# GuidoManni/BodySLAM

Measured on AMD Instinct MI355X. Metric: frames/sec depth+pose+back-proj, 640x480 seq, higher is better.
Workload: dtype f16

## Files before the change

### bodyslam_amd/_lib.py

```python
from __future__ import annotations

import ctypes as C
import os
from typing import Optional

import torch

_HERE = os.path.dirname(os.path.abspath(__file__))
LIB_PATH = os.environ.get("BODYSLAM_HIP_LIB") or os.path.join(_HERE, "libbodyslam_hip.so")

F32, F16, BF16 = 0, 1, 2
F64 = 3
ACT_NONE, ACT_RELU, ACT_GELU, ACT_SOFTPLUS, ACT_SOFTPLUS_FAST = 0, 1, 2, 3, 4
OUT_PLAIN, OUT_SHUFFLE, OUT_QKV = 0, 1, 2

_TORCH2BS = {torch.float32: F32, torch.float16: F16, torch.bfloat16: BF16}
BS2TORCH = {F32: torch.float32, F16: torch.float16, BF16: torch.bfloat16}


class BodySlamHipError(RuntimeError):
    pass


class GemmDesc(C.Structure):
# ... 70 lines not shown
    "bs_odo_p2p_prepare": [C.c_void_p, C.c_int32, C.c_int32, C.c_int32, C.c_double, C.c_void_p, C.c_void_p],
    "bs_odo_p2p_target": [C.c_void_p, C.c_int32, C.c_int32, C.c_int32, C.c_void_p, C.c_void_p, C.c_void_p],
    "bs_odo_p2p_accumulate": [C.c_void_p, C.c_void_p, C.c_int32, C.c_int32, C.c_void_p, C.c_void_p, C.c_double, C.c_double, C.c_void_p, C.c_void_p,
                              C.c_void_p],
    "bs_odo_p2p_step": [C.c_void_p, C.c_void_p, C.c_int32, C.c_int32, C.c_int32, C.c_void_p, C.c_void_p, C.c_int32, C.c_double, C.c_double, C.c_void_p,
                        C.c_void_p, C.c_void_p],
    "bs_tsdf_extract": [C.c_void_p, C.c_int32, C.c_void_p, C.c_void_p, C.c_int32, C.c_void_p, C.c_int32, C.c_int32, C.c_double, C.c_void_p, C.c_void_p,
                        C.c_void_p, C.c_void_p, C.c_void_p, C.c_void_p],
    "bs_tsdf_mesh": [C.c_void_p, C.c_int32, C.c_void_p, C.c_void_p, C.c_int32, C.c_void_p, C.c_int32, C.c_int32, C.c_double, C.c_void_p, C.c_int32] + [C.c_void_p] * 7,
    "bs_tsdf_raycast": [C.c_void_p, C.c_void_p, C.c_int32, C.c_int32, C.c_int32, C.c_double, C.c_double, C.c_void_p, C.c_void_p, C.c_int32, C.c_void_p,
                        C.c_int32, C.c_int32, C.c_double, C.c_double, C.c_void_p, C.c_void_p, C.c_void_p, C.c_void_p, C.c_void_p],
    "bs_attractor_step": [C.c_void_p] * 4 + [C.c_int32] * 8 + [C.c_void_p],
    "bs_add_resized": [C.c_void_p] * 3 + [C.c_int32] * 7 + [C.c_void_p],
    "bs_mlp2": [C.c_void_p, C.c_int32] + [C.c_void_p] * 5 + [C.c_int32] * 6 + [C.c_void_p],
    "bs_mlp2_add": [C.c_void_p] * 7 + [C.c_int32] * 10 + [C.c_void_p],
    "bs_projector_level": [C.c_void_p] * 10 + [C.c_int32] * 9 + [C.c_void_p],
    "bs_logbinom_depth": [C.c_void_p] * 8 + [C.c_int32] * 5 + [C.c_float, C.c_float, C.c_int32, C.c_void_p],
    "bs_logbinom_depth_ex": [C.c_void_p] * 7 + [C.c_int32] + [C.c_void_p] * 2 + [C.c_int32] * 5 + [C.c_float, C.c_float, C.c_int32, C.c_void_p],
    "bs_small_attention": [C.c_void_p, C.c_void_p, C.c_int32, C.c_int32, C.c_int32, C.c_int32, C.c_void_p],
    "bs_route_argmax": [C.c_void_p, C.c_int32, C.c_void_p, C.c_int32, C.c_void_p],
    "bs_postprocess_depth": [C.c_void_p] * 3 + [C.c_int32] * 6 + [C.c_void_p],
    "bs_cyclepose_im2col": [C.c_void_p] * 3 + [C.c_int32] * 4 + [C.c_void_p],
    "bs_cyclepose_im2col_window": [C.c_void_p] * 3 + [C.c_int32] * 8 + [C.c_void_p],
    "bs_instnorm_relu_nhwc": [C.c_void_p] * 4 + [C.c_int32] * 3 + [C.c_float, C.c_int32, C.c_void_p],
    "bs_avgpool_nhwc": [C.c_void_p, C.c_void_p, C.c_int32, C.c_int32, C.c_int32, C.c_void_p],
    "bs_cyclepose_head": [C.c_void_p] * 12 + [C.c_int32] * 3 + [C.c_void_p],
    "bs_backproject": [C.c_void_p, C.c_int32, C.c_int32, C.c_int32, C.c_void_p, C.c_double, C.c_double] + [C.c_void_p] * 6,
    "bs_pose_chain": [C.c_void_p, C.c_int32, C.c_void_p, C.c_void_p, C.c_void_p],
    "bs_pose_chain_from": [C.c_void_p, C.c_int32, C.c_void_p, C.c_void_p, C.c_void_p],
    "bs_pixel_to_3d": [C.c_void_p, C.c_int64, C.c_void_p, C.c_void_p, C.c_void_p],
    "bs_depth_metrics_workspace": [C.c_int32, C.c_int32, C.c_int32],
    "bs_depth_metrics": [C.c_void_p, C.c_void_p] + [C.c_int32] * 3 + [C.c_double, C.c_double, C.c_int32, C.c_double, C.c_void_p, C.c_int64,
                                                                       C.c_void_p, C.c_void_p],
    "bs_similarity_fit": [C.c_void_p, C.c_void_p, C.c_int64, C.c_int32, C.c_void_p, C.c_int64, C.c_void_p, C.c_void_p],
    "bs_trajectory_metrics": [C.c_void_p, C.c_void_p, C.c_void_p, C.c_int32, C.c_int64, C.c_int32, C.c_int32, C.c_int32, C.c_void_p, C.c_void_p],
    "bs_orb_pyramid": [C.c_void_p, C.c_int32, C.c_int32, C.c_int32, C.c_int32, C.c_void_p, C.c_int32, C.c_int64, C.c_void_p, C.c_void_p, C.c_void_p],
    "bs_orb_fast": [C.c_void_p, C.c_int32, C.c_int32, C.c_int32, C.c_void_p, C.c_int32, C.c_int64, C.c_void_p, C.c_void_p, C.c_void_p],
    "bs_orb_select": [C.c_void_p, C.c_void_p, C.c_void_p, C.c_int32, C.c_int32, C.c_int32, C.c_void_p, C.c_int32, C.c_int64, C.c_void_p,
                      C.c_void_p, C.c_void_p, C.c_void_p, C.c_void_p],
    "bs_orb_describe": [C.c_void_p, C.c_void_p, C.c_int32, C.c_int32, C.c_int32, C.c_void_p, C.c_int32, C.c_int64, C.c_void_p, C.c_void_p,
                        C.c_void_p, C.c_void_p, C.c_void_p, C.c_void_p, C.c_void_p, C.c_void_p],
    "bs_orb_match": [C.c_void_p, C.c_void_p, C.c_int32, C.c_void_p, C.c_void_p, C.c_void_p],
    "bs_orb_displacement": [C.c_void_p, C.c_void_p, C.c_void_p, C.c_void_p, C.c_void_p, C.c_int32, C.c_int32, C.c_int32, C.c_void_p, C.c_int32,
                            C.c_void_p, C.c_void_p],
    "bs_orb_lift": [C.c_void_p, C.c_void_p, C.c_void_p, C.c_int32, C.c_int32, C.c_int32, C.c_void_p, C.c_void_p, C.c_void_p],
    "bs_orb_match_pairs": [C.c_void_p, C.c_void_p, C.c_int32, C.c_void_p, C.c_int32, C.c_void_p, C.c_void_p, C.c_void_p],
# ... 474 lines not shown

def logbinom_depth(last, Eh, bins, w0_last, w2, b2, route, depth, B, H, W, He, We, min_temp, max_temp):
    check(load_library().bs_logbinom_depth(p(last), p(Eh), p(bins), p(w0_last), p(w2), p(b2), p(route), p(depth), B, H, W, He, We,
                                           min_temp, max_temp, dt(last), stream_ptr()), "bs_logbinom_depth")


def small_attention(qkv, out, B, S, nheads):
    check(load_library().bs_small_attention(p(qkv), p(out), B, S, nheads, dt(out), stream_ptr()), "bs_small_attention")


def route_argmax(logits, ld, route, B):
    check(load_library().bs_route_argmax(p(logits), ld, p(route), B, stream_ptr()), "bs_route_argmax")


def postprocess_depth(depth_net, depth_m, depth_u16, B, H, W, nh, nw, flip):
    check(load_library().bs_postprocess_depth(p(depth_net), p(depth_m), p(depth_u16), B, H, W, nh, nw, int(flip), stream_ptr()),
          "bs_postprocess_depth")


def cyclepose_im2col(frames, pairs, out, P, H, W):
    check(load_library().bs_cyclepose_im2col(p(frames), p(pairs), p(out), P, H, W, dt(out), stream_ptr()), "bs_cyclepose_im2col")


def instnorm_relu_nhwc(x, out, out_f32, scratch, P, HW, Cch, eps=1e-5):
    check(load_library().bs_instnorm_relu_nhwc(p(x), p(out), p(out_f32), p(scratch), P, HW, Cch, eps, dt(out), stream_ptr()),
          "bs_instnorm_relu_nhwc")


def avgpool_nhwc(x, out, P, HW, Cch):
    check(load_library().bs_avgpool_nhwc(p(x), p(out), P, HW, Cch, stream_ptr()), "bs_avgpool_nhwc")


def cyclepose_head(pooled, x2, w_skip_pool, w_skip_x2, b_skip, w1, b1, w2, b2, pose7, T, scratch, P, HW, Cch):
    check(load_library().bs_cyclepose_head(p(pooled), p(x2), p(w_skip_pool), p(w_skip_x2), p(b_skip), p(w1), p(b1), p(w2), p(b2),
                                           p(pose7), p(T), p(scratch), P, HW, Cch, stream_ptr()), "bs_cyclepose_head")


def backproject(depth_u16, K4, depth_scale, depth_trunc, poses, xyz, idx, count, scratch, B, H, W):
    Karr = (C.c_double * 4)(*[float(v) for v in K4])
    check(load_library().bs_backproject(p(depth_u16), B, H, W, C.cast(Karr, C.c_void_p), float(depth_scale), float(depth_trunc),
                                        p(poses), p(xyz), p(idx), p(count), p(scratch), stream_ptr()), "bs_backproject")


def pose_chain(t_rel, N, g0, g_abs):
    g0arr = None
    if g0 is not None:
        g0arr = C.cast((C.c_double * 16)(*[float(v) for v in g0]), C.c_void_p)
    check(load_library().bs_pose_chain(p(t_rel), N, g0arr, p(g_abs), stream_ptr()), "bs_pose_chain")
# ... 261 lines not shown
```

### bodyslam_amd/csrc/cyclepose.hip

```cpp
#include "common.h"

namespace bs {

constexpr int CP_CROP = 128;
constexpr int CP_K = 320;

template <typename T, bool SPLIT>
__global__ __launch_bounds__(256) void cp_im2col_kernel(const uint8_t* frames, const int32_t* pairs, T* out, int P, int H, int W,
                                                         int top, int left, int CH, int CW) {
    const int64_t total = (int64_t)P * CH * CW * 54;
    const int64_t gid = (int64_t)blockIdx.x * blockDim.x + threadIdx.x;
    if (gid >= total) return;
    const int slot = (int)(gid % 54);
    const int64_t m = gid / 54;
    T* row = out + m * (SPLIT ? 2 * CP_K : CP_K);
    if (slot >= 49) {
        const int k0 = 294 + (slot - 49) * 6;
        for (int i = 0; i < 6 && k0 + i < CP_K; ++i) {
            row[k0 + i] = T16<T>::from_f32(0.0f);
            if (SPLIT) row[CP_K + k0 + i] = T16<T>::from_f32(0.0f);
        }
        return;
    }
    const int x = (int)(m % CW);
// ... 1 lines not shown
    const int p = (int)(m / ((int64_t)CW * CH));
    const int ky = slot / 7, kx = slot - ky * 7;
    int yy = y + ky - 3, xx = x + kx - 3;
    yy = yy < 0 ? -yy : (yy >= CH ? 2 * CH - 2 - yy : yy);
    xx = xx < 0 ? -xx : (xx >= CW ? 2 * CW - 2 - xx : xx);
    const int f0 = pairs[2 * p], f1 = pairs[2 * p + 1];
    const uint8_t* p0 = frames + (((int64_t)f0 * H + top + yy) * W + left + xx) * 3;
    const uint8_t* p1 = frames + (((int64_t)f1 * H + top + yy) * W + left + xx) * 3;
    T* o = row + slot * 6;
#pragma unroll
    for (int c = 0; c < 3; ++c) {
        const float v0 = (__fdiv_rn((float)p0[c], 255.0f) - 0.5f) / 0.5f, v1 = (__fdiv_rn((float)p1[c], 255.0f) - 0.5f) / 0.5f;
        o[c] = T16<T>::from_f32(v0);
        o[3 + c] = T16<T>::from_f32(v1);
        if (SPLIT) {
            o[CP_K + c] = T16<T>::from_f32(v0 - T16<T>::to_f32(o[c]));
            o[CP_K + 3 + c] = T16<T>::from_f32(v1 - T16<T>::to_f32(o[3 + c]));
        }
    }
}

constexpr int IN_CHUNK = 256;

__global__ __launch_bounds__(256) void instnorm_stats_kernel(const float* x, float* part, int HW, int C, int nchunk) {
    const int p = blockIdx.y, ch = blockIdx.x;
    const int tpr = C >> 2, rps = 256 / tpr;
    const int c4 = (threadIdx.x % tpr) * 4, rg = threadIdx.x / tpr;
    const int r0 = ch * IN_CHUNK, r1 = min(HW, r0 + IN_CHUNK);
    const float* xp = x + ((int64_t)p * HW) * C + c4;
    __shared__ float red[256 * 4];
    __shared__ float mean_s[256];
    f32x4 s = {0, 0, 0, 0};
    for (int r = r0 + rg; r < r1; r += rps) {
        const f32x4 v = *reinterpret_cast<const f32x4*>(xp + (int64_t)r * C);
        s += v;
    }
    *reinterpret_cast<f32x4*>(red + threadIdx.x * 4) = s;
    __syncthreads();
    if (threadIdx.x < C) {
        const int c = threadIdx.x;
        float a = 0.f;
        for (int g = 0; g < rps; ++g) a += red[(g * tpr + (c >> 2)) * 4 + (c & 3)];
        mean_s[c] = a / (float)(r1 - r0);
    }
    __syncthreads();
    const f32x4 mu = *reinterpret_cast<const f32x4*>(mean_s + c4);
    f32x4 q = {0, 0, 0, 0};
    for (int r = r0 + rg; r < r1; r += rps) {
        const f32x4 v = *reinterpret_cast<const f32x4*>(xp + (int64_t)r * C) - mu;
        q += v * v;
    }
    __syncthreads();
    *reinterpret_cast<f32x4*>(red + threadIdx.x * 4) = q;
    __syncthreads();
    if (threadIdx.x < C) {
        const int c = threadIdx.x;
        float a = 0.f;
        for (int g = 0; g < rps; ++g) a += red[(g * tpr + (c >> 2)) * 4 + (c & 3)];
        float* o = part + (((int64_t)p * nchunk + ch) * 2) * C;
        o[c] = mean_s[c];
        o[C + c] = a;
    }
}

template <typename T, bool SPLIT>
__global__ __launch_bounds__(256) void instnorm_apply_kernel(const float* x, const float* part, T* out, float* out_f32, int HW, int C,
                                                              int nchunk, float eps) {
    const int p = blockIdx.y, ch = blockIdx.x;
    const int tpr = C >> 2, rps = 256 / tpr;
    const int c4 = (threadIdx.x % tpr) * 4, rg = threadIdx.x / tpr;
    const int r0 = ch * IN_CHUNK, r1 = min(HW, r0 + IN_CHUNK);
    __shared__ float mean_s[256], rstd_s[256];
    if (threadIdx.x < C) {
        const int c = threadIdx.x;
        const float* pp = part + ((int64_t)p * nchunk * 2) * C + c;
        float msum = 0.f;
        for (int k = 0; k < nchunk; ++k) msum += pp[(int64_t)k * 2 * C] * (float)(min(HW, (k + 1) * IN_CHUNK) - k * IN_CHUNK);
        const float mean = msum / (float)HW;
        float m2 = 0.f;
        for (int k = 0; k < nchunk; ++k) {
            const float d = pp[(int64_t)k * 2 * C] - mean;
            m2 += pp[(int64_t)k * 2 * C + C] + d * d * (float)(min(HW, (k + 1) * IN_CHUNK) - k * IN_CHUNK);
        }
        mean_s[c] = mean;
        rstd_s[c] = 1.0f / sqrtf(m2 / (float)HW + eps);
// ... 2 lines not shown
    const f32x4 mu = *reinterpret_cast<const f32x4*>(mean_s + c4), rs = *reinterpret_cast<const f32x4*>(rstd_s + c4);
    const int64_t base = ((int64_t)p * HW) * C + c4;
    for (int r = r0 + rg; r < r1; r += rps) {
        const f32x4 v = *reinterpret_cast<const f32x4*>(x + base + (int64_t)r * C);
        f32x4 y;
        typename T16<T>::v4 o, ol;
#pragma unroll
        for (int e = 0; e < 4; ++e) {
            y[e] = fmaxf((v[e] - mu[e]) * rs[e], 0.0f);
            o[e] = T16<T>::from_f32(y[e]);
            ol[e] = T16<T>::from_f32(y[e] - T16<T>::to_f32(o[e]));
        }
        if (SPLIT) {
            T* op = out + (((int64_t)p * HW + r) * 2) * C + c4;
            *reinterpret_cast<typename T16<T>::v4*>(op) = o;
            *reinterpret_cast<typename T16<T>::v4*>(op + C) = ol;
        } else {
            *reinterpret_cast<typename T16<T>::v4*>(out + base + (int64_t)r * C) = o;
        }
        if (out_f32) *reinterpret_cast<f32x4*>(out_f32 + base + (int64_t)r * C) = y;
    }
}

__global__ __launch_bounds__(256) void avgpool_kernel(const float* x, float* out, int HW, int C) {
    const int p = blockIdx.y, c = blockIdx.x * 64 + (threadIdx.x & 63), g = threadIdx.x >> 6;
    const float* xp = x + (int64_t)p * HW * C + c;
    __shared__ float red[4][64];
    float s = 0.f;
    for (int i = g; i < HW; i += 4) s += xp[(int64_t)i * C];
    red[g][threadIdx.x & 63] = s;
    __syncthreads();
    if (g == 0) {
        const int l = threadIdx.x;
        out[(int64_t)p * C + c] = (red[0][l] + red[1][l] + red[2][l] + red[3][l]) / (float)HW;
    }
}

constexpr int SKIP_CHUNK = 4096;
__global__ __launch_bounds__(256) void skip_partial_kernel(const float* x2, const float* w, float* partial, int K, int nchunk) {
    const int chunk = blockIdx.x, p = blockIdx.y;
    const int k0 = chunk * SKIP_CHUNK;
    const float* xp = x2 + (int64_t)p * K + k0;
    float acc[7] = {0, 0, 0, 0, 0, 0, 0};
    for (int i = threadIdx.x * 4; i < SKIP_CHUNK && k0 + i < K; i += 256 * 4) {
        const f32x4 xv = *reinterpret_cast<const f32x4*>(xp + i);
#pragma unroll
// ... 39 lines not shown
        float skip = 0.f;
        for (int k = 0; k < CP; ++k) skip += w_skip_pool[(int64_t)lane * CP + k] * pv[k];
        for (int c = 0; c < nchunk; ++c) skip += partial[((int64_t)p * nchunk + c) * 8 + lane];
        skip += b_skip[lane];
        out7[lane] = dense + skip;
        pose7[(int64_t)p * 7 + lane] = dense + skip;
    }
    __syncthreads();
    if (lane == 0) {
        const float tx = out7[0], ty = out7[1], tz = out7[2];
        float r = out7[3], i = out7[4], j = out7[5], k = out7[6];
        const float nrm = sqrtf(r * r + i * i + j * j + k * k);
        r /= nrm; i /= nrm; j /= nrm; k /= nrm;
        const float two_s = 2.0f / (r * r + i * i + j * j + k * k);
        float* T = Tout + (int64_t)p * 16;
        T[0] = 1 - two_s * (j * j + k * k); T[1] = two_s * (i * j - k * r);     T[2] = two_s * (i * k + j * r);      T[3] = tx;
        T[4] = two_s * (i * j + k * r);     T[5] = 1 - two_s * (i * i + k * k); T[6] = two_s * (j * k - i * r);      T[7] = ty;
        T[8] = two_s * (i * k - j * r);     T[9] = two_s * (j * k + i * r);     T[10] = 1 - two_s * (i * i + j * j); T[11] = tz;
        T[12] = 0.f; T[13] = 0.f; T[14] = 0.f; T[15] = 1.f;
    }
}

}

static int im2col_launch(const uint8_t* frames, const int32_t* pairs, void* out, int P, int H, int W, int top, int left, int CH, int CW,
                         int dtype, bool split, hipStream_t st) {
    using namespace bs;
    const int64_t total = (int64_t)P * CH * CW * 54;
    const unsigned blocks = (unsigned)cdiv64(total, 256);
    if (dtype == BS_F16 && split)
        hipLaunchKernelGGL((cp_im2col_kernel<f16, true>), dim3(blocks), dim3(256), 0, st, frames, pairs, (f16*)out, P, H, W, top, left, CH, CW);
    else if (dtype == BS_F16)
        hipLaunchKernelGGL((cp_im2col_kernel<f16, false>), dim3(blocks), dim3(256), 0, st, frames, pairs, (f16*)out, P, H, W, top, left, CH, CW);
    else if (split)
        hipLaunchKernelGGL((cp_im2col_kernel<bf16, true>), dim3(blocks), dim3(256), 0, st, frames, pairs, (bf16*)out, P, H, W, top, left, CH, CW);
    else
        hipLaunchKernelGGL((cp_im2col_kernel<bf16, false>), dim3(blocks), dim3(256), 0, st, frames, pairs, (bf16*)out, P, H, W, top, left, CH, CW);
    BS_CHECK_LAUNCH();
    return BS_OK;
}

extern "C" int bs_cyclepose_im2col(const uint8_t* frames, const int32_t* pairs, void* out, int32_t P, int32_t H, int32_t W,
                                   int32_t dtype, void* stream) {
    using namespace bs;
    if (!initialized()) { set_error("bs_cyclepose_im2col: call bs_init first"); return BS_ERR_NOT_INIT; }
    BS_REQUIRE(frames && pairs && out && P >= 0, "bs_cyclepose_im2col: bad argument");
    BS_REQUIRE(H >= CP_CROP && W >= CP_CROP, "bs_cyclepose_im2col: frame %dx%d smaller than the 128 crop", W, H);
    const bool split = (dtype & 16) != 0;
    dtype &= 15;
    BS_REQUIRE(dtype == BS_F16 || dtype == BS_BF16, "bs_cyclepose_im2col: dtype");
    if (P == 0) return BS_OK;
    auto pyround_half = [](int v) { const int q = v / 2; return (v % 2 == 0) ? q : ((q % 2 == 0) ? q : q + 1); };
    const int top = pyround_half(H - CP_CROP), left = pyround_half(W - CP_CROP);
    return im2col_launch(frames, pairs, out, P, H, W, top, left, CP_CROP, CP_CROP, dtype, split, reinterpret_cast<hipStream_t>(stream));
}

extern "C" int bs_cyclepose_im2col_window(const uint8_t* frames, const int32_t* pairs, void* out, int32_t P, int32_t H, int32_t W,
                                          int32_t top, int32_t left, int32_t CH, int32_t CW, int32_t dtype, void* stream) {
    using namespace bs;
    if (!initialized()) { set_error("bs_cyclepose_im2col_window: call bs_init first"); return BS_ERR_NOT_INIT; }
    BS_REQUIRE(frames && pairs && out && P >= 0, "bs_cyclepose_im2col_window: bad argument");
    BS_REQUIRE(CH >= 4 && CW >= 4 && top >= 0 && left >= 0 && top + CH <= H && left + CW <= W,
               "bs_cyclepose_im2col_window: window %dx%d at (%d,%d) outside the %dx%d frame (or smaller than the reflection pad)", CW, CH, left, top, W, H);
    const bool split = (dtype & 16) != 0;
    dtype &= 15;
    BS_REQUIRE(dtype == BS_F16 || dtype == BS_BF16, "bs_cyclepose_im2col_window: dtype");
    if (P == 0) return BS_OK;
    return im2col_launch(frames, pairs, out, P, H, W, top, left, CH, CW, dtype, split, reinterpret_cast<hipStream_t>(stream));
}

extern "C" int bs_instnorm_relu_nhwc(const float* x, void* out, float* out_f32, float* scratch, int32_t P, int32_t HW, int32_t C,
                                     float eps, int32_t dtype, void* stream) {
    using namespace bs;
    if (!initialized()) { set_error("bs_instnorm_relu_nhwc: call bs_init first"); return BS_ERR_NOT_INIT; }
    BS_REQUIRE(x && out && scratch && P >= 0 && HW > 0 && C % 4 == 0 && C >= 4 && C <= 256 && 256 % (C / 4) == 0,
               "bs_instnorm_relu_nhwc: bad argument (C must be 4..256 with C/4 dividing 256)");
    const bool split = (dtype & 16) != 0;
    dtype &= 15;
    BS_REQUIRE(dtype == BS_F16 || dtype == BS_BF16, "bs_instnorm_relu_nhwc: dtype");
    if (P == 0) return BS_OK;
    hipStream_t st = reinterpret_cast<hipStream_t>(stream);
    const int nchunk = cdiv(HW, IN_CHUNK);
    dim3 grid(nchunk, P);
    hipLaunchKernelGGL(instnorm_stats_kernel, grid, dim3(256), 0, st, x, scratch, HW, C, nchunk);
    BS_CHECK_LAUNCH();
    if (dtype == BS_F16 && split)
        hipLaunchKernelGGL((instnorm_apply_kernel<f16, true>), grid, dim3(256), 0, st, x, (const float*)scratch, (f16*)out, out_f32, HW, C, nchunk, eps);
    else if (dtype == BS_F16)
        hipLaunchKernelGGL((instnorm_apply_kernel<f16, false>), grid, dim3(256), 0, st, x, (const float*)scratch, (f16*)out, out_f32, HW, C, nchunk, eps);
    else if (split)
        hipLaunchKernelGGL((instnorm_apply_kernel<bf16, true>), grid, dim3(256), 0, st, x, (const float*)scratch, (bf16*)out, out_f32, HW, C, nchunk, eps);
    else
        hipLaunchKernelGGL((instnorm_apply_kernel<bf16, false>), grid, dim3(256), 0, st, x, (const float*)scratch, (bf16*)out, out_f32, HW, C, nchunk, eps);
    BS_CHECK_LAUNCH();
    return BS_OK;
}

extern "C" int bs_avgpool_nhwc(const float* x, float* out, int32_t P, int32_t HW, int32_t C, void* stream) {
    using namespace bs;
    if (!initialized()) { set_error("bs_avgpool_nhwc: call bs_init first"); return BS_ERR_NOT_INIT; }
    BS_REQUIRE(x && out && P >= 0 && HW > 0 && C % 64 == 0, "bs_avgpool_nhwc: bad argument");
    if (P == 0) return BS_OK;
    hipLaunchKernelGGL(avgpool_kernel, dim3(C / 64, P), dim3(256), 0, reinterpret_cast<hipStream_t>(stream), x, out, HW, C);
    BS_CHECK_LAUNCH();
    return BS_OK;
}

extern "C" int bs_cyclepose_head(const float* pooled, const float* x2, const float* w_skip_pool, const float* w_skip_x2,
// ... 19 lines not shown
```

### bodyslam_amd/csrc/engine.hip

```cpp
#include <stdio.h>
#include <string.h>

#include <exception>
#include <map>
#include <string>
#include <tuple>
#include <type_traits>
#include <utility>
#include <memory>
#include <vector>

#include "common.h"

namespace {

constexpr char kMagic[8] = {'B', 'S', 'E', 'N', 'G', '0', '2', '\0'};
enum { KIND_WORKSPACE = 0, KIND_ZERO = 1, KIND_DATA = 2 };
enum { ARG_I64 = 0, ARG_F64 = 1, ARG_PTR = 2, ARG_NULL = 3, ARG_DESC = 4 };
enum { OP_CALL = 0, OP_SIGNAL = 1, OP_WAIT = 2 };

struct Arg {
    int64_t i = 0;
    double d = 0.0;
    void* p = nullptr;
// ... 20 lines not shown
    static_assert(sizeof...(Args) >= 1, "an entry point takes the stream last");
    Entry e;
    e.nargs = (int)sizeof...(Args) - 1;
    e.fn = reinterpret_cast<const void*>(fn);
    e.thunk = [](const void* f, const Arg* args, void* st) {
        return call_unpacked<Args...>(reinterpret_cast<int (*)(Args...)>(const_cast<void*>(f)), args, st, std::make_index_sequence<sizeof...(Args) - 1>{});
    };
    return e;
}
#define BS_ENGINE_ENTRY(name) {#name, make_entry(name)}
const std::map<std::string, Entry>& entries() {
    static const std::map<std::string, Entry> m = {
        BS_ENGINE_ENTRY(bs_gemm),           BS_ENGINE_ENTRY(bs_attention),          BS_ENGINE_ENTRY(bs_attention_table),
        BS_ENGINE_ENTRY(bs_attention_table_corr),
        BS_ENGINE_ENTRY(bs_layernorm),      BS_ENGINE_ENTRY(bs_cast),               BS_ENGINE_ENTRY(bs_copy_f32),
        BS_ENGINE_ENTRY(bs_cast_split),     BS_ENGINE_ENTRY(bs_relu_split),         BS_ENGINE_ENTRY(bs_preprocess_patches),
        BS_ENGINE_ENTRY(bs_fill_rows),      BS_ENGINE_ENTRY(bs_upconv_tapsum),      BS_ENGINE_ENTRY(bs_small_attention),
        BS_ENGINE_ENTRY(bs_route_argmax),   BS_ENGINE_ENTRY(bs_resize_bilinear_nhwc), BS_ENGINE_ENTRY(bs_rank1_bias),
        BS_ENGINE_ENTRY(bs_postprocess_depth), BS_ENGINE_ENTRY(bs_logbinom_depth_ex), BS_ENGINE_ENTRY(bs_col_mean),
        BS_ENGINE_ENTRY(bs_attractor_step), BS_ENGINE_ENTRY(bs_add_resized),        BS_ENGINE_ENTRY(bs_instnorm_relu_nhwc),
        BS_ENGINE_ENTRY(bs_cyclepose_im2col), BS_ENGINE_ENTRY(bs_cyclepose_im2col_window), BS_ENGINE_ENTRY(bs_cyclepose_head),
        BS_ENGINE_ENTRY(bs_avgpool_nhwc),   BS_ENGINE_ENTRY(bs_mlp2),            BS_ENGINE_ENTRY(bs_mlp2_add),
        BS_ENGINE_ENTRY(bs_upconv_fused),   BS_ENGINE_ENTRY(bs_resize_bias_relu_nhwc), BS_ENGINE_ENTRY(bs_projector_level),
    };
    return m;
}

struct Op {
    int kind = OP_CALL, lane = 0;
    const Entry* entry = nullptr;
    std::vector<Arg> args;
    std::vector<char> desc;
    std::string name;
};
struct Io {
    void* ptr;
    int64_t nbytes;
};

}

struct bs_engine {
    int device = 0;
    std::vector<void*> bufs;
    std::vector<Op> ops;
    std::map<std::string, Io> io;
// ... 305 lines not shown
```

### bodyslam_amd/cyclepose.py

```python
from __future__ import annotations

from typing import Dict, Optional

import torch

from . import _lib as L

CROP = 128
K0 = 320
SKIP_FEATURES = 512 + 256 * 32 * 32


class CyclePoseEngine:
    def __init__(self, weights: Dict[str, torch.Tensor], dtype=torch.float16, device: int = 0, precision: str = "accurate"):
        L.init(device)
        assert dtype in (torch.float16, torch.bfloat16) and precision in ("accurate", "fast")
        self.dtype = dtype
        self.acc = precision == "accurate"
        self.dev = torch.device("cuda", device)
        self._plans = {}
        g = lambda k: weights[k].detach().float()
        h = lambda t: t.to(self.dev, dtype=dtype).contiguous()
        f = lambda t: t.to(self.dev, dtype=torch.float32).contiguous()
        cw = lambda t: t.permute(0, 2, 3, 1).reshape(t.shape[0], -1)

        def split(t):
            hi = t.to(dtype)
            return hi, (t - hi.float()).to(dtype)

        w = self.w = {}
        w0 = cw(g("initial_model.1.weight"))
        w0 = torch.cat([w0, torch.zeros(w0.shape[0], K0 - w0.shape[1])], 1)
        if self.acc:
            hi, lo = split(w0)
            w["c0.w"] = torch.cat([hi, hi, lo], 1).to(self.dev).contiguous()
        else:
            w["c0.w"] = h(w0)
        w["c0.b"] = f(g("initial_model.1.bias"))
        for name, key in (("c1", "downsampling.0"), ("c2", "downsampling.3"), ("c3", "pose_conv.0")):
            k = g(key + ".weight").permute(0, 2, 3, 1)
            if self.acc:
# ... 62 lines not shown
                          f"being applied to a {(h2, w2)} one: same flattened size, other geometry (the reference's Linear would do the same)")
        skip_pool, skip_x2, skip_b = eng._skip[h2 * w2]
        H1, W1 = (CH - 1) // 2 + 1, (CW - 1) // 2 + 1
        H3, W3 = (h2 - 1) // 2 + 1, (w2 - 1) // 2 + 1
        e16 = lambda *s: torch.empty(*s, device=dev, dtype=dt_)
        e32 = lambda *s: torch.empty(*s, device=dev, dtype=torch.float32)
        self.frames = torch.empty(N, H, W, 3, device=dev, dtype=torch.uint8)
        self.pairs = torch.zeros(P, 2, device=dev, dtype=torch.int32)
        Pl = self.plan = L.Plan(dev)
        in_scratch = e32(P * ((CH * CW + 255) // 256) * 2 * 256)
        acc = eng.acc
        m2, SP = (2, 16) if acc else (1, 0)

        def conv(name, A, out, hin, win, ci, co, **kw):
            ho, wo = (hin - 1) // 2 + 1, (win - 1) // 2 + 1
            if acc:
                Pl.gemm(name, A, w[name + ".w"], out, M=P * ho * wo, N=co, K=9 * ci * 3, lda=2 * ci, seg1=ci,
                        conv=(hin, win, 2 * ci, ho, wo, 3, 3, 2, 1, 1), bias=w[name + ".b"],
                        precision_passes=3, **kw)
            else:
                Pl.gemm(name, A, w[name + ".w"], out, M=P * ho * wo, N=co, K=9 * ci, lda=ci,
                        conv=(hin, win, ci, ho, wo, 3, 3, 2, 1, 1), bias=w[name + ".b"], **kw)

        cols = e16(P * CH * CW, K0 * m2)
        if window is None:
            Pl.add("im2col", "bs_cyclepose_im2col", self.frames, self.pairs, cols, P, H, W, L.dt(cols) | SP)
        else:
            Pl.add("im2col", "bs_cyclepose_im2col_window", self.frames, self.pairs, cols, P, H, W, window[0], window[1], CH, CW, L.dt(cols) | SP)
        c0 = e32(P, CH, CW, 64)
        Pl.gemm("c0", cols, w["c0.w"], c0, M=P * CH * CW, N=64, K=K0 * (3 if acc else 1), lda=K0 * m2, seg1=K0 if acc else 0,
                bias=w["c0.b"], precision_passes=3 if acc else 1)
        a0 = e16(P, CH, CW, 64 * m2)
        Pl.add("in0", "bs_instnorm_relu_nhwc", c0, a0, None, in_scratch, P, CH * CW, 64, 1e-5, L.dt(a0) | SP)
        Pl.mark("c0", a0, ("nhwc", P, CH, CW, 64, 1 if acc else 0))
        c1 = e32(P, H1, W1, 128)
        conv("c1", a0, c1, CH, CW, 64, 128)
        a1 = e16(P, H1, W1, 128 * m2)
        Pl.add("in1", "bs_instnorm_relu_nhwc", c1, a1, None, in_scratch, P, H1 * W1, 128, 1e-5, L.dt(a1) | SP)
        c2 = e32(P, h2, w2, 256)
        conv("c2", a1, c2, H1, W1, 128, 256)
        a2 = e16(P, h2, w2, 256 * m2)
        x2 = e32(P, h2, w2, 256)
        Pl.add("in2", "bs_instnorm_relu_nhwc", c2, a2, x2, in_scratch, P, h2 * w2, 256, 1e-5, L.dt(a2) | SP)
        Pl.mark("c2", x2, ("nhwc", P, h2, w2, 256))
        c3 = e32(P, H3, W3, 512)
        conv("c3", a2, c3, h2, w2, 256, 512, act=L.ACT_RELU)
        pooled = e32(P, 512)
        Pl.add("pool", "bs_avgpool_nhwc", c3, pooled, P, H3 * W3, 512)
        Pl.mark("pooled", pooled, ("raw",))
        self.pose7 = e32(P, 7)
        self.T = e32(P, 16)
        scratch = e32(P * ((h2 * w2 * 256 + 4095) // 4096) * 8)
        Pl.add("head", "bs_cyclepose_head", pooled, x2, skip_pool, skip_x2, skip_b, w["d1.w"], w["d1.b"], w["d2.w"], w["d2.b"],
               self.pose7, self.T, scratch, P, h2 * w2, 256)
```

### include/bodyslam_hip.h

```cpp
#ifndef BODYSLAM_HIP_H
#define BODYSLAM_HIP_H

#include <stdint.h>

#ifdef __cplusplus
extern "C" {
#endif

typedef enum {
    BS_OK = 0,
    BS_ERR_INVALID = -1,
    BS_ERR_HIP = -2,
    BS_ERR_NOT_INIT = -3
} bs_status;

enum { BS_F32 = 0, BS_F16 = 1, BS_BF16 = 2, BS_F64 = 3  };
enum { BS_ACT_NONE = 0, BS_ACT_RELU = 1, BS_ACT_GELU = 2, BS_ACT_SOFTPLUS = 3, BS_ACT_SOFTPLUS_FAST = 4 };
enum { BS_OUT_PLAIN = 0, BS_OUT_SHUFFLE = 1, BS_OUT_QKV = 2 };

int bs_init(int device);
const char* bs_last_error(void);
int bs_version(void);

#define BS_F8_ACT_HI_EXP 0
// ... 101 lines not shown
                void* stream);
int bs_projector_level(const void* z, const float* b_c1, const void* emb_prev, const void* Wc2, const float* b_c2, const void* We,
                       const float* b_e, void* x_out, void* emb_out, float* eh_out, int32_t B, int32_t Hl, int32_t Wl, int32_t H, int32_t W,
                       int32_t PM, int32_t E, int32_t NE, int32_t dtype, void* stream);
int bs_add_resized(const void* x, const void* prev, void* out, int32_t B, int32_t Hp, int32_t Wp, int32_t H,
                   int32_t W, int32_t C, int32_t dtype, void* stream);
int bs_logbinom_depth(const void* last, const float* Eh, const float* bins, const float* w0_last, const float* w2,
                      const float* b2, const int32_t* route, float* depth, int32_t B, int32_t H, int32_t W,
                      int32_t He, int32_t We, float min_temp, float max_temp, int32_t dtype, void* stream);
int bs_logbinom_depth_ex(const void* last, const float* Eh, const float* bins, const float* w0_last, const float* w2,
                         const float* b2, const float* rel_w, int32_t hid, const int32_t* route, float* depth, int32_t B,
                         int32_t H, int32_t W, int32_t He, int32_t We, float min_temp, float max_temp, int32_t dtype,
                         void* stream);
int bs_small_attention(const float* qkv, void* out, int32_t B, int32_t S, int32_t nheads, int32_t dtype, void* stream);
int bs_route_argmax(const float* logits, int32_t ld, int32_t* route, int32_t B, void* stream);

int bs_postprocess_depth(const float* depth_net, float* depth_m, uint16_t* depth_u16, int32_t B, int32_t H,
                         int32_t W, int32_t nh, int32_t nw, int32_t flip, void* stream);

int bs_cyclepose_im2col(const uint8_t* frames, const int32_t* pairs, void* out, int32_t P, int32_t H, int32_t W,
                        int32_t dtype, void* stream);
int bs_cyclepose_im2col_window(const uint8_t* frames, const int32_t* pairs, void* out, int32_t P, int32_t H, int32_t W,
                               int32_t top, int32_t left, int32_t CH, int32_t CW, int32_t dtype, void* stream);
int bs_instnorm_relu_nhwc(const float* x, void* out, float* out_f32, float* scratch, int32_t P, int32_t HW, int32_t C,
                          float eps, int32_t dtype, void* stream);
int bs_avgpool_nhwc(const float* x, float* out, int32_t P, int32_t HW, int32_t C, void* stream);
int bs_cyclepose_head(const float* pooled, const float* x2, const float* w_skip_pool, const float* w_skip_x2,
                      const float* b_skip, const float* w1, const float* b1, const float* w2, const float* b2,
                      float* pose7, float* T, float* scratch , int32_t P,
                      int32_t HW, int32_t C, void* stream);

int bs_backproject(const uint16_t* depth, int32_t B, int32_t H, int32_t W, const double* K_host, double depth_scale,
                   double depth_trunc, const double* poses, float* xyz, int32_t* idx, int32_t* count,
                   int32_t* scratch, void* stream);
int bs_pixel_to_3d(const double* uvd, int64_t n, const double* K_host, double* out, void* stream);
int bs_pose_chain(const float* t_rel, int32_t N, const double* g0_host, double* g_abs, void* stream);
int bs_pose_chain_from(const float* t_rel, int32_t N, const double* g0_dev, double* g_abs, void* stream);

#define BS_TSDF_BATCH_MAX 64
#define BS_TSDF_FRAME_BYTES 256
int bs_tsdf_frames_upload(const float* const* depth, const uint8_t* const* color, const double* K, const double* extrinsics, const double* poses,
                          int32_t n_frames, void* frames_dev, void* stream);
int bs_tsdf_touch_batch(const void* frames_dev, int32_t n_frames, int32_t H, int32_t W, int32_t stride, double unit_length, double sdf_trunc,
                        void* table_keys, void* table_fmask, int32_t table_cap, int32_t* counters, void* stream);
int bs_tsdf_integrate_batch(const void* frames_dev, int32_t n_frames, int32_t H, int32_t W, const void* table_keys, int32_t* table_slots,
                            void* table_fmask, int32_t table_cap, int32_t* unit_index, int32_t max_units, int32_t* counters, int32_t* touched,
// ... 159 lines not shown
```

Measured before the change: 495.5.

## Fuse CyclePose first conv im2col, GEMM and instnorm stats into one kernel

Adds a direct convolution kernel for the first CyclePose layer. It builds the normalized, reflection-padded input window in LDS, runs MFMA against double-buffered weight tiles, adds bias, writes the fp32 output and computes per-chunk instance-norm statistics in the same pass. The instnorm launcher can now skip its stats kernel when those statistics are already present. This removes the materialized im2col buffer and its global round trip, plus one kernel launch. In exchange it adds a large LDS footprint and a custom GEMM that may be slower than the tuned generic one.

```diff
diff --git a/bodyslam_amd/_lib.py b/bodyslam_amd/_lib.py
--- a/bodyslam_amd/_lib.py
+++ b/bodyslam_amd/_lib.py
@@ -116,6 +116,8 @@
     "bs_postprocess_depth": [C.c_void_p] * 3 + [C.c_int32] * 6 + [C.c_void_p],
     "bs_cyclepose_im2col": [C.c_void_p] * 3 + [C.c_int32] * 4 + [C.c_void_p],
     "bs_cyclepose_im2col_window": [C.c_void_p] * 3 + [C.c_int32] * 8 + [C.c_void_p],
+    "bs_cyclepose_conv0": [C.c_void_p] * 6 + [C.c_int32] * 8 + [C.c_void_p],
+    "bs_cyclepose_conv0_fits": [C.c_int32] * 3,
     "bs_instnorm_relu_nhwc": [C.c_void_p] * 4 + [C.c_int32] * 3 + [C.c_float, C.c_int32, C.c_void_p],
     "bs_avgpool_nhwc": [C.c_void_p, C.c_void_p, C.c_int32, C.c_int32, C.c_int32, C.c_void_p],
     "bs_cyclepose_head": [C.c_void_p] * 12 + [C.c_int32] * 3 + [C.c_void_p],
@@ -636,8 +638,21 @@
     check(load_library().bs_cyclepose_im2col(p(frames), p(pairs), p(out), P, H, W, dt(out), stream_ptr()), "bs_cyclepose_im2col")
 
 
-def instnorm_relu_nhwc(x, out, out_f32, scratch, P, HW, Cch, eps=1e-5):
-    check(load_library().bs_instnorm_relu_nhwc(p(x), p(out), p(out_f32), p(scratch), P, HW, Cch, eps, dt(out), stream_ptr()),
+def cyclepose_im2col_window(frames, pairs, out, P, H, W, window, split=False):
+    check(load_library().bs_cyclepose_im2col_window(p(frames), p(pairs), p(out), P, H, W, *window, dt(out) | (16 if split else 0), stream_ptr()),
+          "bs_cyclepose_im2col_window")
+
+
+def cyclepose_conv0(frames, pairs, w, bias, out, part, P, H, W, window=None, split=False):
+    top, left, CH, CW = (-1, -1, 128, 128) if window is None else window
+    assert w.shape == (64, 960 if split else 320) and w.is_contiguous() and bias.dtype == torch.float32 and out.dtype == torch.float32
+    check(load_library().bs_cyclepose_conv0(p(frames), p(pairs), p(w), p(bias), p(out), p(part), P, H, W, top, left, CH, CW,
+                                            dt(w) | (16 if split else 0), stream_ptr()), "bs_cyclepose_conv0")
+
+
+def instnorm_relu_nhwc(x, out, out_f32, scratch, P, HW, Cch, eps=1e-5, split=False, have_stats=False):
+    check(load_library().bs_instnorm_relu_nhwc(p(x), p(out), p(out_f32), p(scratch), P, HW, Cch, eps,
+                                               dt(out) | (16 if split else 0) | (32 if have_stats else 0), stream_ptr()),
           "bs_instnorm_relu_nhwc")
 
 
diff --git a/bodyslam_amd/csrc/cyclepose.hip b/bodyslam_amd/csrc/cyclepose.hip
--- a/bodyslam_amd/csrc/cyclepose.hip
+++ b/bodyslam_amd/csrc/cyclepose.hip
@@ -47,17 +47,13 @@
 
 constexpr int IN_CHUNK = 256;
 
-__global__ __launch_bounds__(256) void instnorm_stats_kernel(const float* x, float* part, int HW, int C, int nchunk) {
-    const int p = blockIdx.y, ch = blockIdx.x;
+template <typename Load1, typename Load2>
+__device__ __forceinline__ void in_chunk_stats(Load1 load1, Load2 load2, int r0, int r1, int C, float* red, float* mean_s, float* o) {
     const int tpr = C >> 2, rps = 256 / tpr;
     const int c4 = (threadIdx.x % tpr) * 4, rg = threadIdx.x / tpr;
-    const int r0 = ch * IN_CHUNK, r1 = min(HW, r0 + IN_CHUNK);
-    const float* xp = x + ((int64_t)p * HW) * C + c4;
-    __shared__ float red[256 * 4];
-    __shared__ float mean_s[256];
     f32x4 s = {0, 0, 0, 0};
     for (int r = r0 + rg; r < r1; r += rps) {
-        const f32x4 v = *reinterpret_cast<const f32x4*>(xp + (int64_t)r * C);
+        const f32x4 v = load1(r);
         s += v;
     }
     *reinterpret_cast<f32x4*>(red + threadIdx.x * 4) = s;
@@ -72,7 +68,7 @@
     const f32x4 mu = *reinterpret_cast<const f32x4*>(mean_s + c4);
     f32x4 q = {0, 0, 0, 0};
     for (int r = r0 + rg; r < r1; r += rps) {
-        const f32x4 v = *reinterpret_cast<const f32x4*>(xp + (int64_t)r * C) - mu;
+        const f32x4 v = load2(r) - mu;
         q += v * v;
     }
     __syncthreads();
@@ -82,10 +78,20 @@
         const int c = threadIdx.x;
         float a = 0.f;
         for (int g = 0; g < rps; ++g) a += red[(g * tpr + (c >> 2)) * 4 + (c & 3)];
-        float* o = part + (((int64_t)p * nchunk + ch) * 2) * C;
         o[c] = mean_s[c];
         o[C + c] = a;
     }
+}
+
+__global__ __launch_bounds__(256) void instnorm_stats_kernel(const float* x, float* part, int HW, int C, int nchunk) {
+    const int p = blockIdx.y, ch = blockIdx.x;
+    const int c4 = (threadIdx.x % (C >> 2)) * 4;
+    const int r0 = ch * IN_CHUNK, r1 = min(HW, r0 + IN_CHUNK);
+    const float* xp = x + ((int64_t)p * HW) * C + c4;
+    __shared__ float red[256 * 4];
+    __shared__ float mean_s[256];
+    auto load = [&](int r) { return *reinterpret_cast<const f32x4*>(xp + (int64_t)r * C); };
+    in_chunk_stats(load, load, r0, r1, C, red, mean_s, part + (((int64_t)p * nchunk + ch) * 2) * C);
 }
 
 template <typename T, bool SPLIT>
@@ -134,6 +140,136 @@
     }
 }
 
+constexpr int C0_WBUF = 64 * 128;
+constexpr int C0_TSTRIDE = 68;
+constexpr int C0_TILE_BYTES = IN_CHUNK * C0_TSTRIDE * 4;
+constexpr int C0_LDS_MAX = 128 * 1024;
+
+template <typename T, bool SPLIT>
+__global__ __launch_bounds__(256) void cp_conv0_kernel(const uint8_t* frames, const int32_t* pairs, const T* w, const float* bias, float* out,
+                                                        float* part, int H, int W, int top, int left, int CH, int CW, int nchunk) {
+    typedef typename T16<T>::v8 v8;
+    extern __shared__ __attribute__((aligned(16))) char smem[];
+    __shared__ float red[256 * 4];
+    __shared__ float mean_s[64];
+    constexpr int KT = SPLIT ? 3 * CP_K : CP_K;
+    constexpr int NT = KT / 64;
+    const int ch = blockIdx.x, p = blockIdx.y;
+    const int tid = threadIdx.x, lane = tid & 63, wave = tid >> 6;
+    const int HW = CH * CW;
+    const int r0 = ch * IN_CHUNK, r1 = min(HW, r0 + IN_CHUNK);
+    const int y0 = r0 / CW, y1 = (r1 - 1) / CW;
+    const int SW = CW + 6, nsy = y1 - y0 + 7;
+    const int plane = nsy * SW * 6;
+    T* whi = reinterpret_cast<T*>(smem + 2 * C0_WBUF);
+    T* wlo = whi + plane;
+
+    const int wrow = tid >> 3, wpos = ((tid & 7) ^ (wrow & 7)) * 16;
+    const char* wsrc = reinterpret_cast<const char*>(w) + (size_t)wrow * (KT * 2) + (tid & 7) * 16;
+    u32x4 wr[2];
+    auto w_load = [&](int t) {
+#pragma unroll
+        for (int j = 0; j < 2; ++j) wr[j] = *reinterpret_cast<const u32x4*>(wsrc + (size_t)j * 32 * (KT * 2) + t * 128);
+    };
+    auto w_store = [&](int buf) {
+#pragma unroll
+        for (int j = 0; j < 2; ++j) *reinterpret_cast<u32x4*>(smem + buf * C0_WBUF + (wrow + j * 32) * 128 + wpos) = wr[j];
+    };
+    w_load(0);
+    {
+        const int f0 = pairs[2 * p], f1 = pairs[2 * p + 1];
+        for (int it = tid; it < nsy * SW * 2; it += 256) {
+            const int f = it & 1, s = it >> 1;
+            const int sy = s / SW, sx = s - sy * SW;
+            int yy = y0 + sy - 3, xx = sx - 3;
+            yy = yy < 0 ? -yy : (yy >= CH ? 2 * CH - 2 - yy : yy);
+            xx = xx < 0 ? -xx : (xx >= CW ? 2 * CW - 2 - xx : xx);
+            const uint8_t* px = frames + (((int64_t)(f ? f1 : f0) * H + top + yy) * W + left + xx) * 3;
+            T* o = whi + s * 6 + f * 3;
+#pragma unroll
+            for (int c = 0; c < 3; ++c) {
+                const float v = (__fdiv_rn((float)px[c], 255.0f) - 0.5f) / 0.5f;
+                o[c] = T16<T>::from_f32(v);
+                if (SPLIT) o[plane + c] = T16<T>::from_f32(v - T16<T>::to_f32(o[c]));
+            }
+        }
+    }
+    w_store(0);
+    __syncthreads();
+
+    const int frow = lane & 15, fq = lane >> 4;
+    int abase[4];
+#pragma unroll
+    for (int i = 0; i < 4; ++i) {
+        const int r = min(r0 + wave * 64 + i * 16 + frow, r1 - 1);
+        const int y = r / CW, x = r - y * CW;
+        abase[i] = ((y - y0) * SW + x) * 6;
+    }
+    const int wfrag = frow * 128, wswz = frow & 7;
+    f32x4 acc[4][4];
+#pragma unroll
+    for (int i = 0; i < 4; ++i)
+#pragma unroll
+        for (int j = 0; j < 4; ++j) acc[i][j] = f32x4{0.f, 0.f, 0.f, 0.f};
+    for (int t = 0; t < NT; ++t) {
+        if (t + 1 < NT) w_load(t + 1);
+        const int seg = t / 5, kt = (t - seg * 5) * 64;
+        const T* pl = (SPLIT && seg == 1) ? wlo : whi;
+        const char* sb = smem + (t & 1) * C0_WBUF;
+#pragma unroll
+        for (int kk = 0; kk < 2; ++kk) {
+            int off[4];
+            bool live[4];
+#pragma unroll
+            for (int e = 0; e < 4; ++e) {
+                const int k = kt + kk * 32 + fq * 8 + 2 * e;
+                const int ky = k / 42;
+                live[e] = k < 294;
+                off[e] = live[e] ? ky * (SW * 6) + (k - ky * 42) : 0;
+            }
+            v8 af[4], bf[4];
+#pragma unroll
+            for (int i = 0; i < 4; ++i) {
+                u32x4 d;
+#pragma unroll
+                for (int e = 0; e < 4; ++e) {
+                    const uint32_t v = *reinterpret_cast<const uint32_t*>(pl + abase[i] + off[e]);
+                    d[e] = live[e] ? v : 0u;
+                }
+                af[i] = __builtin_bit_cast(v8, d);
+            }
+#pragma unroll
+            for (int j = 0; j < 4; ++j) bf[j] = *reinterpret_cast<const v8*>(sb + j * 16 * 128 + wfrag + (((kk * 4 + fq) ^ wswz) << 4));
+#pragma unroll
+            for (int i = 0; i < 4; ++i)
+#pragma unroll
+                for (int j = 0; j < 4; ++j) acc[i][j] = T16<T>::mfma16(bf[j], af[i], acc[i][j]);
+        }
+        if (t + 1 < NT) w_store((t + 1) & 1);
+        __syncthreads();
+    }
+
+    float* tile = reinterpret_cast<float*>(smem);
+#pragma unroll
+    for (int j = 0; j < 4; ++j) {
+        const f32x4 bj = *reinterpret_cast<const f32x4*>(bias + j * 16 + fq * 4);
+#pragma unroll
+        for (int i = 0; i < 4; ++i)
+            *reinterpret_cast<f32x4*>(tile + (wave * 64 + i * 16 + frow) * C0_TSTRIDE + j * 16 + fq * 4) = acc[i][j] + bj;
+    }
+    __syncthreads();
+
+    const int c4 = (tid & 15) * 4;
+    float* op = out + ((int64_t)p * HW) * 64 + c4;
+    auto load1 = [&](int r) {
+        const f32x4 v = *reinterpret_cast<const f32x4*>(tile + (r - r0) * C0_TSTRIDE + c4);
+        *reinterpret_cast<f32x4*>(op + (int64_t)r * 64) = v;
+        return v;
+    };
+    auto load2 = [&](int r) { return *reinterpret_cast<const f32x4*>(tile + (r - r0) * C0_TSTRIDE + c4); };
+    in_chunk_stats(load1, load2, r0, r1, 64, red, mean_s, part + (((int64_t)p * nchunk + ch) * 2) * 64);
+}
+
 __global__ __launch_bounds__(256) void avgpool_kernel(const float* x, float* out, int HW, int C) {
     const int p = blockIdx.y, c = blockIdx.x * 64 + (threadIdx.x & 63), g = threadIdx.x >> 6;
     const float* xp = x + (int64_t)p * HW * C + c;
@@ -219,6 +355,8 @@
 }
 
 }
+
+static int pyround_half(int v) { const int q = v / 2; return (v % 2 == 0) ? q : ((q % 2 == 0) ? q : q + 1); }
 
 static int im2col_launch(const uint8_t* frames, const int32_t* pairs, void* out, int P, int H, int W, int top, int left, int CH, int CW,
                          int dtype, bool split, hipStream_t st) {
@@ -247,7 +385,6 @@
     dtype &= 15;
     BS_REQUIRE(dtype == BS_F16 || dtype == BS_BF16, "bs_cyclepose_im2col: dtype");
     if (P == 0) return BS_OK;
-    auto pyround_half = [](int v) { const int q = v / 2; return (v % 2 == 0) ? q : ((q % 2 == 0) ? q : q + 1); };
     const int top = pyround_half(H - CP_CROP), left = pyround_half(W - CP_CROP);
     return im2col_launch(frames, pairs, out, P, H, W, top, left, CP_CROP, CP_CROP, dtype, split, reinterpret_cast<hipStream_t>(stream));
 }
@@ -266,6 +403,55 @@
     return im2col_launch(frames, pairs, out, P, H, W, top, left, CH, CW, dtype, split, reinterpret_cast<hipStream_t>(stream));
 }
 
+static int64_t conv0_lds_bytes(int CH, int CW, bool split) {
+    using namespace bs;
+    int rows = (IN_CHUNK % CW == 0) ? IN_CHUNK / CW : (IN_CHUNK - 2) / CW + 2;
+    rows = (rows < CH ? rows : CH) + 6;
+    const int64_t win = (int64_t)rows * (CW + 6) * 6 * 2 * (split ? 2 : 1) + 2 * C0_WBUF;
+    return win > C0_TILE_BYTES ? win : C0_TILE_BYTES;
+}
+
+extern "C" int bs_cyclepose_conv0_fits(int32_t CH, int32_t CW, int32_t dtype) {
+    if (CH < 4 || CW < 4) return 0;
+    return conv0_lds_bytes(CH, CW, (dtype & 16) != 0) <= bs::C0_LDS_MAX ? 1 : 0;
+}
+
+template <typename T, bool SPLIT>
+static int conv0_launch(const uint8_t* frames, const int32_t* pairs, const void* w, const float* bias, float* out, float* part, int P, int H, int W,
+                        int top, int left, int CH, int CW, hipStream_t st) {
+    using namespace bs;
+    BS_MAX_DYNAMIC_LDS(reinterpret_cast<const void*>(cp_conv0_kernel<T, SPLIT>), C0_LDS_MAX);
+    const int nchunk = cdiv(CH * CW, IN_CHUNK);
+    hipLaunchKernelGGL((cp_conv0_kernel<T, SPLIT>), dim3(nchunk, P), dim3(256), (size_t)conv0_lds_bytes(CH, CW, SPLIT), st, frames, pairs, (const T*)w,
+                       bias, out, part, H, W, top, left, CH, CW, nchunk);
+    BS_CHECK_LAUNCH();
+    return BS_OK;
+}
+
+extern "C" int bs_cyclepose_conv0(const uint8_t* frames, const int32_t* pairs, const void* w, const float* bias, float* out, float* part,
+                                  int32_t P, int32_t H, int32_t W, int32_t top, int32_t left, int32_t CH, int32_t CW, int32_t dtype, void* stream) {
+    using namespace bs;
+    if (!initialized()) { set_error("bs_cyclepose_conv0: call bs_init first"); return BS_ERR_NOT_INIT; }
+    BS_REQUIRE(frames && pairs && w && bias && out && part && P >= 0 && P <= 65535, "bs_cyclepose_conv0: bad argument");
+    if (top < 0) {
+        BS_REQUIRE(CH == CP_CROP && CW == CP_CROP && H >= CP_CROP && W >= CP_CROP, "bs_cyclepose_conv0: the centre crop is 128 x 128 of a frame at least that large");
+        top = pyround_half(H - CP_CROP);
+        left = pyround_half(W - CP_CROP);
+    }
+    BS_REQUIRE(CH >= 4 && CW >= 4 && left >= 0 && top + CH <= H && left + CW <= W && (int64_t)CH * CW < (1ll << 31) - IN_CHUNK,
+               "bs_cyclepose_conv0: window %dx%d at (%d,%d) outside the %dx%d frame (or smaller than the reflection pad)", CW, CH, left, top, W, H);
+    const bool split = (dtype & 16) != 0;
+    dtype &= 15;
+    BS_REQUIRE(dtype == BS_F16 || dtype == BS_BF16, "bs_cyclepose_conv0: dtype");
+    BS_REQUIRE(conv0_lds_bytes(CH, CW, split) <= C0_LDS_MAX, "bs_cyclepose_conv0: a %d-wide window does not fit the LDS (bs_cyclepose_conv0_fits)", CW);
+    if (P == 0) return BS_OK;
+    hipStream_t st = reinterpret_cast<hipStream_t>(stream);
+    if (dtype == BS_F16 && split) return conv0_launch<f16, true>(frames, pairs, w, bias, out, part, P, H, W, top, left, CH, CW, st);
+    if (dtype == BS_F16) return conv0_launch<f16, false>(frames, pairs, w, bias, out, part, P, H, W, top, left, CH, CW, st);
+    if (split) return conv0_launch<bf16, true>(frames, pairs, w, bias, out, part, P, H, W, top, left, CH, CW, st);
+    return conv0_launch<bf16, false>(frames, pairs, w, bias, out, part, P, H, W, top, left, CH, CW, st);
+}
+
 extern "C" int bs_instnorm_relu_nhwc(const float* x, void* out, float* out_f32, float* scratch, int32_t P, int32_t HW, int32_t C,
                                      float eps, int32_t dtype, void* stream) {
     using namespace bs;
@@ -273,14 +459,17 @@
     BS_REQUIRE(x && out && scratch && P >= 0 && HW > 0 && C % 4 == 0 && C >= 4 && C <= 256 && 256 % (C / 4) == 0,
                "bs_instnorm_relu_nhwc: bad argument (C must be 4..256 with C/4 dividing 256)");
     const bool split = (dtype & 16) != 0;
+    const bool have_stats = (dtype & 32) != 0;
     dtype &= 15;
     BS_REQUIRE(dtype == BS_F16 || dtype == BS_BF16, "bs_instnorm_relu_nhwc: dtype");
     if (P == 0) return BS_OK;
     hipStream_t st = reinterpret_cast<hipStream_t>(stream);
     const int nchunk = cdiv(HW, IN_CHUNK);
     dim3 grid(nchunk, P);
-    hipLaunchKernelGGL(instnorm_stats_kernel, grid, dim3(256), 0, st, x, scratch, HW, C, nchunk);
-    BS_CHECK_LAUNCH();
+    if (!have_stats) {
+        hipLaunchKernelGGL(instnorm_stats_kernel, grid, dim3(256), 0, st, x, scratch, HW, C, nchunk);
+        BS_CHECK_LAUNCH();
+    }
     if (dtype == BS_F16 && split)
         hipLaunchKernelGGL((instnorm_apply_kernel<f16, true>), grid, dim3(256), 0, st, x, (const float*)scratch, (f16*)out, out_f32, HW, C, nchunk, eps);
     else if (dtype == BS_F16)
diff --git a/bodyslam_amd/csrc/engine.hip b/bodyslam_amd/csrc/engine.hip
--- a/bodyslam_amd/csrc/engine.hip
+++ b/bodyslam_amd/csrc/engine.hip
@@ -66,6 +66,7 @@
         BS_ENGINE_ENTRY(bs_cyclepose_im2col), BS_ENGINE_ENTRY(bs_cyclepose_im2col_window), BS_ENGINE_ENTRY(bs_cyclepose_head),
         BS_ENGINE_ENTRY(bs_avgpool_nhwc),   BS_ENGINE_ENTRY(bs_mlp2),            BS_ENGINE_ENTRY(bs_mlp2_add),
         BS_ENGINE_ENTRY(bs_upconv_fused),   BS_ENGINE_ENTRY(bs_resize_bias_relu_nhwc), BS_ENGINE_ENTRY(bs_projector_level),
+        BS_ENGINE_ENTRY(bs_cyclepose_conv0),
     };
     return m;
 }
diff --git a/bodyslam_amd/cyclepose.py b/bodyslam_amd/cyclepose.py
--- a/bodyslam_amd/cyclepose.py
+++ b/bodyslam_amd/cyclepose.py
@@ -12,11 +12,13 @@
 
 
 class CyclePoseEngine:
-    def __init__(self, weights: Dict[str, torch.Tensor], dtype=torch.float16, device: int = 0, precision: str = "accurate"):
+    def __init__(self, weights: Dict[str, torch.Tensor], dtype=torch.float16, device: int = 0, precision: str = "accurate",
+                 direct_c0: bool = True):
         L.init(device)
         assert dtype in (torch.float16, torch.bfloat16) and precision in ("accurate", "fast")
         self.dtype = dtype
         self.acc = precision == "accurate"
+        self.direct_c0 = bool(direct_c0)
         self.dev = torch.device("cuda", device)
         self._plans = {}
         g = lambda k: weights[k].detach().float()
@@ -125,16 +127,23 @@
                 Pl.gemm(name, A, w[name + ".w"], out, M=P * ho * wo, N=co, K=9 * ci, lda=ci,
                         conv=(hin, win, ci, ho, wo, 3, 3, 2, 1, 1), bias=w[name + ".b"], **kw)
 
-        cols = e16(P * CH * CW, K0 * m2)
-        if window is None:
-            Pl.add("im2col", "bs_cyclepose_im2col", self.frames, self.pairs, cols, P, H, W, L.dt(cols) | SP)
+        c0 = e32(P, CH, CW, 64)
+        a0 = e16(P, CH, CW, 64 * m2)
+        self.direct_c0 = eng.direct_c0 and bool(L.load_library().bs_cyclepose_conv0_fits(CH, CW, L.dt(a0) | SP))
+        if self.direct_c0:
+            top, left = (-1, -1) if window is None else (window[0], window[1])
+            Pl.add("c0", "bs_cyclepose_conv0", self.frames, self.pairs, w["c0.w"], w["c0.b"], c0, in_scratch, P, H, W, top, left, CH, CW,
+                   L.dt(a0) | SP)
+            Pl.add("in0", "bs_instnorm_relu_nhwc", c0, a0, None, in_scratch, P, CH * CW, 64, 1e-5, L.dt(a0) | SP | 32)
         else:
-            Pl.add("im2col", "bs_cyclepose_im2col_window", self.frames, self.pairs, cols, P, H, W, window[0], window[1], CH, CW, L.dt(cols) | SP)
-        c0 = e32(P, CH, CW, 64)
-        Pl.gemm("c0", cols, w["c0.w"], c0, M=P * CH * CW, N=64, K=K0 * (3 if acc else 1), lda=K0 * m2, seg1=K0 if acc else 0,
-                bias=w["c0.b"], precision_passes=3 if acc else 1)
-        a0 = e16(P, CH, CW, 64 * m2)
-        Pl.add("in0", "bs_instnorm_relu_nhwc", c0, a0, None, in_scratch, P, CH * CW, 64, 1e-5, L.dt(a0) | SP)
+            cols = e16(P * CH * CW, K0 * m2)
+            if window is None:
+                Pl.add("im2col", "bs_cyclepose_im2col", self.frames, self.pairs, cols, P, H, W, L.dt(cols) | SP)
+            else:
+                Pl.add("im2col", "bs_cyclepose_im2col_window", self.frames, self.pairs, cols, P, H, W, window[0], window[1], CH, CW, L.dt(cols) | SP)
+            Pl.gemm("c0", cols, w["c0.w"], c0, M=P * CH * CW, N=64, K=K0 * (3 if acc else 1), lda=K0 * m2, seg1=K0 if acc else 0,
+                    bias=w["c0.b"], precision_passes=3 if acc else 1)
+            Pl.add("in0", "bs_instnorm_relu_nhwc", c0, a0, None, in_scratch, P, CH * CW, 64, 1e-5, L.dt(a0) | SP)
         Pl.mark("c0", a0, ("nhwc", P, CH, CW, 64, 1 if acc else 0))
         c1 = e32(P, H1, W1, 128)
         conv("c1", a0, c1, CH, CW, 64, 128)
diff --git a/include/bodyslam_hip.h b/include/bodyslam_hip.h
--- a/include/bodyslam_hip.h
+++ b/include/bodyslam_hip.h
@@ -147,6 +147,9 @@
                         int32_t dtype, void* stream);
 int bs_cyclepose_im2col_window(const uint8_t* frames, const int32_t* pairs, void* out, int32_t P, int32_t H, int32_t W,
                                int32_t top, int32_t left, int32_t CH, int32_t CW, int32_t dtype, void* stream);
+int bs_cyclepose_conv0(const uint8_t* frames, const int32_t* pairs, const void* w, const float* bias, float* out, float* part,
+                       int32_t P, int32_t H, int32_t W, int32_t top, int32_t left, int32_t CH, int32_t CW, int32_t dtype, void* stream);
+int bs_cyclepose_conv0_fits(int32_t CH, int32_t CW, int32_t dtype);
 int bs_instnorm_relu_nhwc(const float* x, void* out, float* out_f32, float* scratch, int32_t P, int32_t HW, int32_t C,
                           float eps, int32_t dtype, void* stream);
 int bs_avgpool_nhwc(const float* x, float* out, int32_t P, int32_t HW, int32_t C, void* stream);
```

After: 499.3 (median of 6 runs). About the same (+0.8%).
